# prashantraina/neural_raytracing

Measured on NVIDIA B200. Metric: rays_per_sec, higher is better.
Workload: dtype f16

## Files before the change

### neural_raytracing_b200/csrc/nrt_tc.cu

```cuda
#include <stdlib.h>

#include "tc_core.cuh"
#include "camera_math.cuh"

namespace tc {

template <int IN, int LAT, int OUT>
struct IoPlain {
  const float* x; const float* latent; float* out; int out_act;
  __device__ __forceinline__ void load(int64_t m, float* v) const {
#pragma unroll
    for (int j = 0; j < IN; ++j) v[j] = __ldg(x + m * IN + j);
#pragma unroll
    for (int j = 0; j < LAT; ++j) v[IN + j] = __ldg(latent + m * LAT + j);
  }
  __device__ __forceinline__ void store(int64_t m, const float* o) const {
#pragma unroll
    for (int j = 0; j < OUT; ++j) {
      float v = o[j];
      if (out_act == NRT_OUT_SIGMOID) v = 1.0f / (1.0f + __expf(-v));
      else if (out_act == NRT_OUT_SOFTPLUS) v = v > 20.0f ? v : __logf(1.0f + __expf(v));
      else if (out_act == NRT_OUT_TANH) v = tanhf(v);
      out[m * OUT + j] = v;
    }
  }
};

static inline int pow2_shift(int S) { int k = 0; while ((1 << k) < S) ++k; return (1 << k) == S ? k : -1; }
__device__ __forceinline__ int64_t ray_of(int64_t m, int S, int shift) { return shift >= 0 ? (m >> shift) : m / S; }

struct NoCam {};
struct WithCam { nrtcam::CamDev cam; int64_t r_off; };

template <int NLAT, bool CAM = false>
struct IoNerfFirst {
  const float* rays; const float* ts; const float* ts_per_ray; int S;
  float* sigma; void* latent; int fmt; int lat32; int s_shift;
  std::conditional_t<CAM, WithCam, NoCam> c;
  __device__ __forceinline__ void load(int64_t m, float* v) const {
    const int64_t ray = ray_of(m, S, s_shift);
    const int s = (int)(m - ray * S);
    const float t = ts_per_ray ? __ldg(ts_per_ray + m) : __ldg(ts + s);
    if constexpr (CAM) {
      float o[3], d[3];
      int view;
      nrtcam::cam_ray(c.cam, c.r_off + ray, o, d, &view);
      v[0] = o[0] + t * d[0]; v[1] = o[1] + t * d[1]; v[2] = o[2] + t * d[2];
    } else {
      const float* r = rays + ray * 6;
      v[0] = __ldg(r) + t * __ldg(r + 3);
      v[1] = __ldg(r + 1) + t * __ldg(r + 4);
      v[2] = __ldg(r + 2) + t * __ldg(r + 5);
    }
  }
  __device__ __forceinline__ void store(int64_t m, const float* o) const {
    sigma[m] = o[0];
    if (lat32) {
      float4* dst = reinterpret_cast<float4*>(latent) + (m >> 7) * (int64_t)(NLAT / 4 * 128) + (m & 127);
#pragma unroll
      for (int j = 0; j < NLAT / 4; ++j) dst[j * 128] = make_float4(o[1 + 4 * j], o[2 + 4 * j], o[3 + 4 * j], o[4 + 4 * j]);
      return;
    }
    uint4* dst = reinterpret_cast<uint4*>(latent) + (m >> 7) * (int64_t)(NLAT / 8 * 128) + (m & 127);
#pragma unroll
    for (int j = 0; j < NLAT / 8; ++j) {
      uint4 q;
      if (fmt == 0) {
        q.x = Elem<0>::pack(o[1 + 8 * j], o[2 + 8 * j]); q.y = Elem<0>::pack(o[3 + 8 * j], o[4 + 8 * j]);
        q.z = Elem<0>::pack(o[5 + 8 * j], o[6 + 8 * j]); q.w = Elem<0>::pack(o[7 + 8 * j], o[8 + 8 * j]);
      } else {
        q.x = Elem<1>::pack(o[1 + 8 * j], o[2 + 8 * j]); q.y = Elem<1>::pack(o[3 + 8 * j], o[4 + 8 * j]);
        q.z = Elem<1>::pack(o[5 + 8 * j], o[6 + 8 * j]); q.w = Elem<1>::pack(o[7 + 8 * j], o[8 + 8 * j]);
      }
      dst[j * 128] = q;
    }
  }
};

template <int NLAT, int LD, bool PACKED = false, bool CAM = false>
struct IoNerfSecond {
  const float* rays; const void* latent; const float* light_code; const int32_t* view_of_ray; int S;
  float* rgb; int fmt; int out_act; int lat32; int s_shift;
  std::conditional_t<CAM, WithCam, NoCam> c;
  __device__ __forceinline__ int dir_and_view(int64_t ray, float* d) const {
    if constexpr (CAM) {
      float o[3];
      int view;
      nrtcam::cam_ray(c.cam, c.r_off + ray, o, d, &view);
      return view;
    } else {
      const float* r = rays + ray * 6;
      d[0] = __ldg(r + 3); d[1] = __ldg(r + 4); d[2] = __ldg(r + 5);
      return view_of_ray ? __ldg(view_of_ray + ray) : 0;
    }
  }
  __device__ __forceinline__ void load(int64_t m, float* v) const {
    const int64_t ray = ray_of(m, S, s_shift);
    if (lat32) {
      const float4* src = reinterpret_cast<const float4*>(latent) + (m >> 7) * (int64_t)(NLAT / 4 * 128) + (m & 127);
#pragma unroll
      for (int j = 0; j < NLAT / 4; ++j) {
        const float4 q = __ldg(src + j * 128);
        v[4 * j] = q.x; v[4 * j + 1] = q.y; v[4 * j + 2] = q.z; v[4 * j + 3] = q.w;
      }
    } else {
      const uint4* src = reinterpret_cast<const uint4*>(latent) + (m >> 7) * (int64_t)(NLAT / 8 * 128) + (m & 127);
#pragma unroll
      for (int j = 0; j < NLAT / 8; ++j) {
        const uint4 q = __ldg(src + j * 128);
        const uint32_t w[4] = {q.x, q.y, q.z, q.w};
#pragma unroll
        for (int e = 0; e < 4; ++e) {
          if (fmt == 0) {
            v[8 * j + 2 * e] = Elem<0>::back((uint16_t)(w[e] & 0xffff)); v[8 * j + 2 * e + 1] = Elem<0>::back((uint16_t)(w[e] >> 16));
          } else {
            v[8 * j + 2 * e] = Elem<1>::back((uint16_t)(w[e] & 0xffff)); v[8 * j + 2 * e + 1] = Elem<1>::back((uint16_t)(w[e] >> 16));
          }
        }
      }
    }
    const int view = dir_and_view(ray, v + NLAT);
#pragma unroll
    for (int j = 0; j < LD; ++j) v[NLAT + 3 + j] = __ldg(light_code + (int64_t)view * LD + j);
  }
  static constexpr int kPackedPairs = PACKED ? NLAT / 2 : 0;
  __device__ __forceinline__ void load_packed(int64_t m, uint32_t* w, float* v) const {
    const int64_t ray = ray_of(m, S, s_shift);
    const uint4* src = reinterpret_cast<const uint4*>(latent) + (m >> 7) * (int64_t)(NLAT / 8 * 128) + (m & 127);
#pragma unroll
    for (int j = 0; j < NLAT / 8; ++j) {
      const uint4 q = __ldg(src + j * 128);
      w[4 * j] = q.x; w[4 * j + 1] = q.y; w[4 * j + 2] = q.z; w[4 * j + 3] = q.w;
    }
    const int view = dir_and_view(ray, v + NLAT);
#pragma unroll
    for (int j = 0; j < LD; ++j) v[NLAT + 3 + j] = __ldg(light_code + (int64_t)view * LD + j);
  }
  __device__ __forceinline__ void store(int64_t m, const float* o) const {
#pragma unroll
    for (int j = 0; j < 3; ++j) {
      float v = o[j];
      if (out_act == NRT_OUT_SIGMOID) v = 1.0f / (1.0f + __expf(-v));
      else if (out_act == NRT_OUT_TANH) v = tanhf(v);
      rgb[m * 3 + j] = v;
    }
  }
};

static long long* g_dbg_timeline = nullptr;
extern "C" void nrtdbg_set_timeline(long long* dev_buf) { g_dbg_timeline = dev_buf; }

#ifndef NRT_SPH_MAX
#define NRT_SPH_MAX 128
#endif
constexpr int kSphMax = NRT_SPH_MAX;
__device__ __forceinline__ float* sph_table() {
  __shared__ __align__(16) float tab[kSphMax * 13];
  return tab;
}
__device__ __forceinline__ void sph_fill(const SdfDev& sd) {
  if (sd.n > kSphMax) return;
  float* tab = sph_table();
  for (int e = threadIdx.x; e < sd.n * 13; e += blockDim.x) {
    const int i = e / 13, k = e - i * 13;
    float v;
    if (k == 12) v = __ldg(sd.radii + i);
    else {
      const int j = k >> 2, c = k & 3;
      v = c == 3 ? __ldg(sd.centers + i * 3 + j) : __ldg(sd.tfs + i * 9 + j * 3 + c) + (j == c ? 1.0f : 0.0f);
    }
    tab[k == 12 ? kSphMax * 12 + i : i * 12 + k] = v;
  }
}
template <bool APPROX = false>
__device__ __forceinline__ float sphere_smin_fast(const SdfDev& sd, float px, float py, float pz) {
  float sum = 0.0f;
  if (sd.n <= kSphMax) {
    const float4* rows = reinterpret_cast<const float4*>(sph_table());
    const float* rad = sph_table() + kSphMax * 12;
#pragma unroll 4
    for (int i = 0; i < sd.n; ++i) {
      const float4 a = rows[i * 3], b = rows[i * 3 + 1], c = rows[i * 3 + 2];
      const float q0 = fmaf(a.z, pz, fmaf(a.y, py, a.x * px)) - a.w;
      const float q1 = fmaf(b.z, pz, fmaf(b.y, py, b.x * px)) - b.w;
      const float q2 = fmaf(c.z, pz, fmaf(c.y, py, c.x * px)) - c.w;
      const float d2 = fmaf(q2, q2, fmaf(q1, q1, q0 * q0));
      if constexpr (APPROX) {
        float rs;
        asm("rsqrt.approx.ftz.f32 %0, %1;" : "=f"(rs) : "f"(fmaxf(d2, 1e-30f)));
        sum += tc::ex2_approx((rad[i] - d2 * rs) * 46.16624130844683f);
      } else {
        const float d = sqrtf(d2) - rad[i];
        sum += __expf(-32.0f * d);
      }
    }
    return -__logf(fmaxf(sum, 1e-4f)) * (1.0f / 32.0f);
  }
  for (int i = 0; i < sd.n; ++i) {
    const float* T = sd.tfs + i * 9;
    float q[3];
#pragma unroll
    for (int j = 0; j < 3; ++j) {
      const float t0 = __ldg(T + j * 3 + 0) + (j == 0 ? 1.0f : 0.0f);
      const float t1 = __ldg(T + j * 3 + 1) + (j == 1 ? 1.0f : 0.0f);
      const float t2 = __ldg(T + j * 3 + 2) + (j == 2 ? 1.0f : 0.0f);
      q[j] = fmaf(t2, pz, fmaf(t1, py, t0 * px)) - __ldg(sd.centers + i * 3 + j);
    }
    const float d = sqrtf(fmaf(q[2], q[2], fmaf(q[1], q[1], q[0] * q[0]))) - __ldg(sd.radii + i);
    sum += __expf(-32.0f * d);
  }
  return -__logf(fmaxf(sum, 1e-4f)) * (1.0f / 32.0f);
}

struct IoSdfEval {
  static constexpr int kSplitOut = 1;
  SdfDev sd; const float* p; float* out;
  __device__ __forceinline__ void cta_init() const { sph_fill(sd); }
  __device__ __forceinline__ void load(int64_t m, float* v) const {
    v[0] = __ldg(p + m * 3); v[1] = __ldg(p + m * 3 + 1); v[2] = __ldg(p + m * 3 + 2);
  }
  __device__ __forceinline__ void store(int64_t m, const float* o) const {
    out[m] = sphere_smin_fast(sd, __ldg(p + m * 3), __ldg(p + m * 3 + 1), __ldg(p + m * 3 + 2)) + o[0];
  }
};

__device__ __forceinline__ long long grab_ray(unsigned long long* counter, int64_t R, bool need) {
  const unsigned bal = __ballot_sync(0xffffffffu, need);
  if (bal == 0) return -1;
  const int lane = threadIdx.x & 31;
  unsigned long long base = 0;
  if (lane == __ffs(bal) - 1) base = atomicAdd(counter, (unsigned long long)__popc(bal));
  base = __shfl_sync(0xffffffffu, base, __ffs(bal) - 1);
  const long long r = (long long)base + __popc(bal & ((1u << lane) - 1u));
// ... 39 lines not shown
          s.d[0] = __ldg(rp + 3); s.d[1] = __ldg(rp + 4); s.d[2] = __ldg(rp + 5);
          s.t = t_start; s.it = 0; s.r = r;
          s.tmax = (MODE == TC_MARCH_SHADOW) ? __ldg(max_t_per_ray + r) : max_t;
        }
      }
    }
    if (s.r < 0) return false;
#pragma unroll
    for (int j = 0; j < 3; ++j) { s.p[j] = __fadd_rn(s.o[j], __fmul_rn(s.d[j], s.t)); x[j] = s.p[j]; }
    return true;
  }
  __device__ __forceinline__ void consume(State& s, const float* o) const {
    const float d = sphere_smin_fast<MODE != TC_MARCH_PRIMARY || ((NRT_MARCH_FAST & 2) != 0)>(sd, s.p[0], s.p[1], s.p[2]) + o[0];
    s.steps++;
    if (MODE == TC_MARCH_PRIMARY) {
      if (d <= eps) { depth[s.r] = s.t; flag[s.r] = 1; s.r = -1; }
      else { s.t += d; s.it++; }
    } else {
      s.t += d; s.it++;
      if (d < eps) { flag[s.r] = (s.t >= s.tmax) ? 1 : 0; s.r = -1; }
    }
  }
  __device__ __forceinline__ void finish(State& s) const {
    if (steps_done == nullptr) return;
    unsigned v = s.steps;
    for (int o = 16; o > 0; o >>= 1) v += __shfl_down_sync(0xffffffffu, v, o);
    if ((threadIdx.x & 31) == 0 && v) atomicAdd(steps_done, (unsigned long long)v);
  }
};

struct IoScanEval {
  static constexpr int kSoftplusForm = 3;
  __device__ __forceinline__ void cta_init() const { sph_fill(sd); }
  SdfDev sd;
  const float* rays; double step; int n1; float* val;
  __device__ __forceinline__ void point(int64_t m, float* p) const {
    const uint32_t ray = (uint32_t)m / (uint32_t)n1;
    const int k = (int)((uint32_t)m - ray * (uint32_t)n1);
    const float* rp = rays + (int64_t)ray * 6;
    const float t = (float)(step * (double)k);
#pragma unroll
    for (int j = 0; j < 3; ++j) p[j] = (k == 0) ? __ldg(rp + j) : __fadd_rn(__ldg(rp + j), __fmul_rn(t, __ldg(rp + 3 + j)));
  }
  __device__ __forceinline__ void load(int64_t m, float* x) const { point(m, x); }
  __device__ __forceinline__ void store(int64_t m, const float* o) const {
    float p[3];
    point(m, p);
    val[m] = sphere_smin_fast<true>(sd, p[0], p[1], p[2]) + o[0];
  }
};
__global__ void k_scan_argmin(const float* __restrict__ val, const float* __restrict__ rays, int64_t R, int n1, double step,
                              int32_t* __restrict__ best_idx, float* __restrict__ best_pos, float* __restrict__ min_val) {
  const int lane = threadIdx.x & 31;
  const int64_t r = ((int64_t)blockIdx.x * blockDim.x + threadIdx.x) >> 5;
  if (r >= R) return;
  const float* v = val + r * n1;
  float best = 3.0e38f;
  int idx = 0x7fffffff;
  for (int k = lane; k < n1; k += 32) {
    const float x = v[k];
    if (x < best) { best = x; idx = k; }
  }
  for (int o = 16; o > 0; o >>= 1) {
    const float ob = __shfl_xor_sync(0xffffffffu, best, o);
    const int oi = __shfl_xor_sync(0xffffffffu, idx, o);
    if (ob < best || (ob == best && oi < idx)) { best = ob; idx = oi; }
  }
  if (lane == 0) {
    best_idx[r] = idx;
    if (min_val) min_val[r] = best;
    const float tb = __fmul_rn((float)idx, (float)step);
    for (int j = 0; j < 3; ++j) best_pos[r * 3 + j] = __fadd_rn(rays[r * 6 + j], __fmul_rn(tb, rays[r * 6 + 3 + j]));
  }
}

template <class NET, class IO, int FMT, class SV = NoSave>
static int launch(const void* blob, const IO& io, int64_t M, cudaStream_t st, int tag = TAG_TC_MLP, SV sv = SV{}) {
  const size_t bytes = (size_t)NET::SMEM_BYTES + 256;
  auto kern = k_mlp_tc<NET, IO, FMT, SV>;
  NRT_CUDA(cudaFuncSetAttribute(kern, cudaFuncAttributeMaxDynamicSharedMemorySize, (int)bytes));
  const int64_t ntiles = (M + 127) / 128;
  const int grid = (int)std::min<int64_t>((ntiles + NET::NSLOT - 1) / NET::NSLOT, (int64_t)nrt_sm_count());
  NrtProfScope _ps(tag, st);
  kern<<<grid, NET::threads(NET::WPS), bytes, st>>>(reinterpret_cast<const uint8_t*>(blob) + NET::BLOB_OFF, io, M, g_dbg_timeline, sv);
  NRT_CUDA(cudaGetLastError());
  return NRT_OK;
}

using NetNerfFirst = Net<3, 0, 16, 128, 5, 3, 65, NRT_ACT_LEAKY_RELU>;
using NetNerfFirstR = Net<3, 0, 16, 128, 5, 3, 65, NRT_ACT_LEAKY_RELU, (NRT_BIAS_MMA & 4) != 0>;
using NetNerfSecondPT = Net<70, 0, 16, 64, 8, 3, 3, NRT_ACT_LEAKY_RELU>;
using NetNerfSecondLE = Net<115, 0, 16, 64, 8, 3, 3, NRT_ACT_LEAKY_RELU>;
using NetNeuralBsdf = Net<3, 0, 64, 96, 6, 3, 3, NRT_ACT_LEAKY_RELU>;
using NetOcc = Net<5, 0, 16, 64, 8, 3, 1, NRT_ACT_LEAKY_RELU>;
using NetPlainFirst = Net<3, 32, 16, 32, 5, 3, 33, NRT_ACT_LEAKY_RELU>;
using NetPlainSecond = Net<2, 64, 16, 32, 5, 3, 3, NRT_ACT_LEAKY_RELU>;
using NetSdfShift = Net<3, 0, 32, 128, 8, 3, 1, NRT_ACT_SOFTPLUS>;

template <class NET>
static bool matches(const MlpDev& d) {
  return d.in_size == NET::IN && d.latent == NET::LAT && d.freqs == NET::F && d.hidden == NET::H && d.L == NET::L &&
         d.skip == NET::SKIP && d.out == NET::OUT && d.act == NET::ACT;
}
template <class NET>
static bool matches(const nrt_mlp_t& m) {
  return m.in_size == NET::IN && m.latent_size == NET::LAT && m.freqs == NET::F && m.hidden == NET::H && m.num_layers == NET::L &&
         m.skip == NET::SKIP && m.out_size == NET::OUT && m.act == NET::ACT;
}

}

using namespace tc;

static int fmt_of(int prec) { return prec == NRT_PREC_BF16 ? 1 : 0; }

extern "C" int64_t nrt_mlp_tc_blob_bytes(const nrt_mlp_t* m, int prec) {
  NRT_REQUIRE(m != nullptr, "mlp descriptor is NULL");
  NRT_REQUIRE(prec == NRT_PREC_F16 || prec == NRT_PREC_BF16, "nrt_mlp_tc_blob_bytes: prec must be F16 or BF16");
  NRT_REQUIRE(m->num_layers >= 1 && m->num_layers <= NRT_MAX_LAYERS && m->hidden % 16 == 0, "unsupported MLP shape");
  if (matches<NetNerfFirst>(*m)) return (int64_t)NetNerfFirstR::BLOB_OFF + NetNerfFirstR::Y.bytes;
  const Layout y = make_layout(m->in_size, m->latent_size, m->freqs, m->hidden, m->num_layers, m->skip, m->out_size);
  return (int64_t)y.bytes;
}

extern "C" int nrt_mlp_pack_tc(const nrt_mlp_t* m, int prec, void* blob_out, void* stream) {
  MlpDev d;
  int rc = nrt_build_mlp_dev(m, &d);
  if (rc != NRT_OK) return rc;
  NRT_REQUIRE(prec == NRT_PREC_F16 || prec == NRT_PREC_BF16, "nrt_mlp_pack_tc: prec must be F16 or BF16");
  NRT_REQUIRE(blob_out != nullptr && ((uintptr_t)blob_out & 15) == 0, "blob_out must be 16-byte aligned");
  NRT_REQUIRE(d.hidden % 16 == 0, "hidden must be a multiple of 16");
  NrtProfScope _ps(TAG_TC_PACK, (cudaStream_t)stream);
  auto pack = [&](const Layout& y, const BiasRows& br, uint8_t* dst) {
    const int grid = std::min(nrt_cdiv(pack_tc_items(y), 256), 1184);
    if (fmt_of(prec) == 0) k_pack_tc<0><<<grid, 256, 0, (cudaStream_t)stream>>>(d, y, br, dst);
    else k_pack_tc<1><<<grid, 256, 0, (cudaStream_t)stream>>>(d, y, br, dst);
  };
  pack(make_layout(d.in_size, d.latent, d.freqs, d.hidden, d.L, d.skip, d.out), no_bias_rows(), (uint8_t*)blob_out);
  if (NetNerfFirstR::BLOB_OFF > 0 && matches<NetNerfFirst>(d))
    pack(NetNerfFirstR::Y, NetNerfFirstR::BR, (uint8_t*)blob_out + NetNerfFirstR::BLOB_OFF);
  NRT_CUDA(cudaGetLastError());
  return NRT_OK;
}

template <class NET>
static int forward_plain(const nrt_mlp_t* m, int prec, int out_act, const float* x, const float* latent, int64_t M,
                         float* out, cudaStream_t st) {
  IoPlain<NET::IN, NET::LAT, NET::OUT> io{x, latent, out, out_act};
  if (fmt_of(prec) == 0) return launch<NET, decltype(io), 0>(m->params_tc, io, M, st);
  return launch<NET, decltype(io), 1>(m->params_tc, io, M, st);
}
template <class NET>
static int forward_plain_save(const nrt_mlp_t* m, int prec, int out_act, const float* x, const float* latent, int64_t M,
                              float* out, float* acts, cudaStream_t st) {
  IoPlain<NET::IN, NET::LAT, NET::OUT> io{x, latent, out, out_act};
  SaveF32 sv{acts, M};
  if (fmt_of(prec) == 0) return launch<NET, decltype(io), 0, SaveF32>(m->params_tc, io, M, st, TAG_TC_MLP, sv);
  return launch<NET, decltype(io), 1, SaveF32>(m->params_tc, io, M, st, TAG_TC_MLP, sv);
}

int nrt_mlp_forward_tc_wide(const nrt_mlp_t* m, const MlpDev& d, int prec, int out_act, const float* x, int64_t M, float* out,
                            float* acts, cudaStream_t st, bool* handled);

int nrt_mlp_forward_tc(const nrt_mlp_t* m, int prec, int out_act, const float* x, const float* latent, int64_t M,
                       float* out, float* acts, cudaStream_t st) {
  MlpDev d;
  int rc = nrt_build_mlp_dev(m, &d);
// ... 192 lines not shown
```

### neural_raytracing_b200/csrc/tc_core.cuh

```cuda
#pragma once
#include <cuda_bf16.h>
#include <cuda_fp16.h>

#include <algorithm>
#include <type_traits>

#include "nrt_common.cuh"

namespace tc {

constexpr int kMaxOps = NRT_MAX_LAYERS + 3;

struct Layout {
  int split, XR, KRAW, KE, KX, KPH, FP, NOP;
  int n_ops;
  int opN[kMaxOps], opK[kMaxOps];
  int op_off[kMaxOps];
  int w_elems;
  int bias_off[kMaxOps];
  int bias_floats;
  int wout_f32_off;
  int basis_f32_off;
  int bytes;
};
// ... 836 lines not shown
#define NRT_MMA_WARP_PER_SLOT_STREAM 0
#endif
#ifndef NRT_SELF_ISSUE
#define NRT_SELF_ISSUE 0
#endif
  static constexpr bool SELF = NRT_SELF_ISSUE != 0 && STREAM && ACT == NRT_ACT_SOFTPLUS && ENC_CUDA && FUSE_OUT && NSLOT == 2;
  static constexpr int NMMA = SELF ? 0 : ((STREAM ? NRT_MMA_WARP_PER_SLOT_STREAM != 0 : NRT_MMA_WARP_PER_SLOT != 0) ? NSLOT : 1);
  static constexpr int threads(int wps) { return NWG * wps * 32 + 32 * NMMA; }
  static constexpr int max_op_bytes() {
    int m = 0;
    for (int o = 0; o < Y.n_ops; ++o) m = imax(m, Y.opN[o] * Y.opK[o] * 2);
    return m;
  }
  static constexpr int MAXOP = max_op_bytes();
  static constexpr int BIAS_BYTES = Y.bias_floats * 4;
  static constexpr int SMEM_BYTES = STREAM ? NSLOT * 2 * MAXOP + BIAS_BYTES : Y.bytes;
  static constexpr bool FITS_SMEM = SMEM_BYTES <= kSmemBudget;
};

constexpr int kEpiThreads = 128;

template <class NET, int FMT, int ST, int PART = 0, bool BMMA = false, int ZLO = 0>
__device__ __forceinline__ void issue_stage(uint32_t b_addr, uint32_t dD, uint32_t aU, uint32_t aE, uint64_t* done_bar) {
  constexpr Layout Y = NET::Y;
  constexpr uint32_t N = (uint32_t)Y.opN[ST];
  constexpr uint32_t idesc = (1u << 4) | ((uint32_t)FMT << 7) | ((uint32_t)FMT << 10) | ((N >> 3) << 17) |
                             ((uint32_t)(128 >> 4) << 24);
  constexpr uint32_t lbo = N * 16, sbo = 128;
  constexpr int kch = Y.opK[ST] / 16;
  constexpr int k_u = (ST >= 2 && ST < NET::STAGES - 1) ? NET::H / 16 : ((NET::INPLACE && ST == 1) ? 0 : kch);
  if (elect_one()) {
    const uint64_t bd0 = make_desc(NET::STREAM ? b_addr : b_addr + (uint32_t)Y.op_off[ST] * 2u, lbo, sbo);
    constexpr bool kBiasChunk = BMMA && !NET::BIAS_ROWS && ST > 0 && ST < NET::END_STAGE;
    constexpr bool kBiasChunk8 = BMMA && NET::BIAS_ROWS && NET::BR.bk8_off[ST] >= 0;
    constexpr bool kFromZero = ST == 0 || (BMMA && NET::BIAS_ROWS && NET::BR.bk8_off[ST] < 0);
    if constexpr (kBiasChunk) {
      static_assert(NET::BIAS_MMA && N == (uint32_t)NET::H, "bias K-chunks: hidden-width MMA layers of a resident blob");
      mma_ts(dD, (uint32_t)NET::ONES_COL, make_desc(b_addr + (uint32_t)NET::BK_OFF + (uint32_t)(ST - 1) * N * 32u, lbo, sbo), idesc, 0u);
    }
    if constexpr (kBiasChunk8) {
      static_assert(!NET::STREAM, "bias chunks of a resident blob");
      mma_ts(dD, (uint32_t)NET::ONES_COL, make_desc(b_addr + (uint32_t)NET::BR.bk8_off[ST] * 2u, lbo, sbo), idesc, 0u);
    }
#pragma unroll
    for (int kc = 0; kc < kch; ++kc) {
      if (PART == 1 && kc >= k_u / 2 && kc < k_u) continue;
      if (PART == 2 && (kc < k_u / 2 || kc >= k_u)) continue;
      uint32_t a;
      if constexpr (ST == 0) {
        constexpr int xch = NET::XR / 16;
        static_assert(ZLO < xch, "the chunk with the non-latent x_lo columns stays");
        if (kc >= xch && kc < xch + ZLO) continue;
        const uint32_t hi = NET::INPLACE ? aE : aU, lo = NET::INPLACE ? aU : aE;
        a = (kc >= xch && kc < 2 * xch) ? (lo + (kc - xch) * 8) : (hi + (kc % xch) * 8);
      } else {
        a = (kc < k_u) ? (aU + kc * 8) : (aE + (kc - k_u) * 8);
      }
      mma_ts(dD, a, bd0 + (uint64_t)((kc * 2 * lbo) >> 4), idesc, (!kFromZero || kc > 0) ? 1u : 0u);
    }
    if (PART != 1) tc_commit(done_bar);
  }
  __syncwarp();
}
template <class NET, int FMT, int PART = 0, bool BMMA = false, int ZLO = 0>
__device__ __forceinline__ void issue_stage_dyn(int st, uint32_t b_addr, uint32_t dD, uint32_t aU, uint32_t aE,
                                                uint64_t* done_bar) {
#define NRT_STAGE_CASE(S) case S: if constexpr (S < NET::STAGES && (PART == 0 || S >= 2)) issue_stage<NET, FMT, S, PART, BMMA, ZLO>(b_addr, dD, aU, aE, done_bar); break;
  switch (st) {
    NRT_STAGE_CASE(0) NRT_STAGE_CASE(1) NRT_STAGE_CASE(2) NRT_STAGE_CASE(3) NRT_STAGE_CASE(4) NRT_STAGE_CASE(5)
    NRT_STAGE_CASE(6) NRT_STAGE_CASE(7) NRT_STAGE_CASE(8) NRT_STAGE_CASE(9) NRT_STAGE_CASE(10) NRT_STAGE_CASE(11)
    NRT_STAGE_CASE(12) NRT_STAGE_CASE(13) NRT_STAGE_CASE(14) NRT_STAGE_CASE(15) NRT_STAGE_CASE(16) NRT_STAGE_CASE(17)
    NRT_STAGE_CASE(18) NRT_STAGE_CASE(19) NRT_STAGE_CASE(20) NRT_STAGE_CASE(21) NRT_STAGE_CASE(22)
    default: break;
  }
#undef NRT_STAGE_CASE
}
__device__ __forceinline__ void stream_op(uint8_t* dst, const uint8_t* src, uint32_t bytes, uint64_t* bar) {
  mbar_expect_tx(bar, bytes);
  for (uint32_t off = 0; off < bytes; off += 32768u) bulk_g2s(dst + off, src + off, min(32768u, bytes - off), bar);
}

template <class T, class = void> struct PackedPairsOf { static constexpr int value = 0; };
template <class T> struct PackedPairsOf<T, std::void_t<decltype(T::kPackedPairs)>> { static constexpr int value = T::kPackedPairs; };
template <class T, class = void> struct HasCtaInit : std::false_type {};
template <class T> struct HasCtaInit<T, std::void_t<decltype(&T::cta_init)>> : std::true_type {};
template <class T, class = void> struct IsIterative : std::false_type {};
template <class T> struct IsIterative<T, std::void_t<typename T::State>> : std::true_type {};
struct NoState {};
template <class T, class = void> struct StateOf { using type = NoState; };
template <class T> struct StateOf<T, std::void_t<typename T::State>> { using type = typename T::State; };

__device__ __forceinline__ void named_bar_sync(int id, int nthreads) {
  asm volatile("bar.sync %0, %1;" ::"r"(id), "r"(nthreads) : "memory");
}

#ifdef NRT_MAXNREG
#define NRT_KMLP_BOUNDS(T) __maxnreg__(((65536 / (T)) / 8 * 8) > 255 ? 255 : ((65536 / (T)) / 8 * 8))
#else
#define NRT_KMLP_BOUNDS(T) __launch_bounds__(T, 1)
#endif
template <class NET, class IO, int FMT, class SV = NoSave, int WPS = NET::WPS>
__global__ void NRT_KMLP_BOUNDS(NET::threads(WPS))
k_mlp_tc(const uint8_t* __restrict__ blob, IO io, int64_t M, long long* __restrict__ dbg, SV sv = SV{}) {
  constexpr int EPI = WPS * 32;
  static_assert(NET::FITS_TMEM, "network does not fit in TMEM");
  static_assert(NET::FITS_SMEM, "stage buffers do not fit in shared memory");
  constexpr int kDbgIt0 = 4, kDbgIts = 4;
  auto stamp = [&](int it, int st, int slot, int k) {
    if (dbg != nullptr && slot < 2 && blockIdx.x == 0 && it >= kDbgIt0 && it < kDbgIt0 + kDbgIts)
      dbg[(((it - kDbgIt0) * NET::STAGES + st) * 2 + slot) * 8 + k] = clock64();
  };
  using E = Elem<FMT>;
  constexpr Layout Y = NET::Y;
  constexpr int H = NET::H, IN = NET::IN, LAT = NET::LAT, F = NET::F, L = NET::L;
  constexpr int NSLOT = NET::NSLOT;
  extern __shared__ __align__(128) uint8_t smem[];
  constexpr bool STREAM = NET::STREAM;
  uint16_t* sW = reinterpret_cast<uint16_t*>(smem);
  const float* sBias = reinterpret_cast<const float*>(smem + (STREAM ? (size_t)NSLOT * 2 * NET::MAXOP : (size_t)Y.w_elems * 2));
  __shared__ __align__(8) uint64_t bar_w;
  __shared__ __align__(8) uint64_t bar_wfull[3][2];
  __shared__ uint32_t s_opoff[NET::STAGES], s_opbytes[NET::STAGES];
  __shared__ __align__(8) uint64_t bar_ready[3];
  __shared__ __align__(8) uint64_t bar_ready_a[3];
  __shared__ __align__(8) uint64_t bar_done[3];
  constexpr bool KSPLIT = NET::KSPLIT && WPS == 4 && !SV::kOn && !SV::kF32;
#ifndef NRT_SOFTPLUS_FULLROW
#define NRT_SOFTPLUS_FULLROW 0
#endif
#ifndef NRT_SOFTPLUS_PIPE
#define NRT_SOFTPLUS_PIPE 1
#endif
  constexpr bool kPipeRow = NRT_SOFTPLUS_PIPE != 0 && SoftplusOf<IO>::value != 0 && NET::ACT == NRT_ACT_SOFTPLUS && !KSPLIT &&
                            !SV::kOn && !SV::kF32;
  constexpr bool kFullRow = NRT_SOFTPLUS_FULLROW != 0 && !kPipeRow && NET::ACT == NRT_ACT_SOFTPLUS && !KSPLIT && !SV::kOn && !SV::kF32;
  __shared__ uint32_t tmem_base_s;
  __shared__ uint32_t s_bias[NET::STAGES];
  constexpr bool ITER = IsIterative<IO>::value;
  constexpr bool BMMA = NET::BIAS_MMA && !KSPLIT && WPS == 4 && !SV::kOn && !SV::kF32;
  static_assert(BMMA || !NET::BIAS_ROWS, "the render layout has no fp32 biases to pre-load");
  constexpr int kPP = (!ITER && !NET::SPLIT && !SV::kOn && !SV::kF32 && LAT == 0 && NET::ACT == NRT_ACT_LEAKY_RELU) ? PackedPairsOf<IO>::value : 0;
  constexpr int ZLO = (NRT_BIAS_MMA & 2) ? 2 * kPP / 16 : 0;
  __shared__ volatile uint32_t s_slot_live[3];
  __shared__ uint32_t s_warp_live[3][4];

  const int tid = threadIdx.x;
  const int warp = tid >> 5;
  constexpr bool SELF = NET::SELF;
  const int mma_id = SELF ? -1 : warp - NET::NWG * WPS;
  const bool is_mma_warp = SELF ? warp == 0 : mma_id == 0;
  __shared__ uint32_t s_issue_lock;
  const int64_t ntiles = (M + 127) / 128;
  if constexpr (HasCtaInit<IO>::value) io.cta_init();
  if (tid < NET::STAGES) {
    s_bias[tid] = (uint32_t)Y.bias_off[tid];
    s_opoff[tid] = (uint32_t)Y.op_off[tid] * 2;
    s_opbytes[tid] = (uint32_t)(Y.opN[tid] * Y.opK[tid] * 2);
  }

  if (tid == 0) {
    s_slot_live[0] = 1; s_slot_live[1] = 1; s_slot_live[2] = 1;
    s_issue_lock = 0;
    mbar_init(&bar_w, 1);
    for (int s = 0; s < 3; ++s) {
      mbar_init(&bar_ready[s], EPI); mbar_init(&bar_done[s], 1); mbar_init(&bar_ready_a[s], EPI);
      mbar_init(&bar_wfull[s][0], 1); mbar_init(&bar_wfull[s][1], 1);
    }
    asm volatile("fence.mbarrier_init.release.cluster;" ::: "memory");
  }
  __syncthreads();
  if (is_mma_warp) {
    asm volatile("tcgen05.alloc.cta_group::1.sync.aligned.shared::cta.b32 [%0], 512;" ::"r"(smem_u32(&tmem_base_s)) : "memory");
    asm volatile("tcgen05.relinquish_alloc_permit.cta_group::1.sync.aligned;" ::: "memory");
    if ((tid & 31) == 0) {
      if (STREAM) {
        mbar_expect_tx(&bar_w, (uint32_t)NET::BIAS_BYTES);
        bulk_g2s(smem + (size_t)NSLOT * 2 * NET::MAXOP, blob + (size_t)Y.w_elems * 2, (uint32_t)NET::BIAS_BYTES, &bar_w);
      } else {
        mbar_expect_tx(&bar_w, (uint32_t)Y.bytes);
        constexpr uint32_t kChunk = 32768;
        for (uint32_t off = 0; off < (uint32_t)Y.bytes; off += kChunk) {
          const uint32_t n = min(kChunk, (uint32_t)Y.bytes - off);
          bulk_g2s(smem + off, blob + off, n, &bar_w);
        }
      }
    }
  }
  tc_fence_before();
  __syncthreads();
  tc_fence_after();
  if (tmem_base_s != 0u) __trap();
  constexpr uint32_t tmem = 0u;
  if constexpr (BMMA) {
    if (warp < 4) {
      const uint32_t one = (uint32_t)one16<FMT>();
      const uint32_t r[8] = {one | (one << 16), one, 0u, 0u, 0u, 0u, 0u, 0u};
      TmemIO<8>::st(tmem + ((uint32_t)(warp * 32) << 16) + (uint32_t)NET::ONES_COL, r);
      tc_wait_st();
    }
    tc_fence_before();
    __syncthreads();
    tc_fence_after();
  }
  mbar_wait(&bar_w, 0);

  if (mma_id >= 0) {
    constexpr int NMMA = NET::NMMA;
    constexpr bool OWN = NMMA == NSLOT;
    auto mine = [&](int slot) { return slot % (NMMA > 0 ? NMMA : 1) == mma_id; };
#ifndef NRT_MMA_ALTERNATE
#define NRT_MMA_ALTERNATE 0
#endif
    constexpr bool ALT = NRT_MMA_ALTERNATE != 0 && !OWN && NSLOT == 2 && !KSPLIT;
    int turn = 0;
    bool live[3];
    auto is_ready = [&](int slot, uint64_t* bar, uint32_t parity) {
      if constexpr (OWN) { mbar_wait(bar, parity); return true; }
      else if constexpr (ALT) {
        if (slot != turn && live[turn]) return false;
        mbar_wait(bar, parity);
        turn = slot ^ 1;
        return true;
      }
      else return mbar_test(bar, parity);
    };
// ... 82 lines not shown
            stream_op(smem + (size_t)(slot * 2 + nb) * NET::MAXOP, blob + s_opoff[st[slot]], s_opbytes[st[slot]],
                      &bar_wfull[slot][nb]);
          }
          __syncwarp();
        }
      }
#ifndef NRT_MMA_POLL_SLEEP_NS
#define NRT_MMA_POLL_SLEEP_NS 0
#endif
      if (NRT_MMA_POLL_SLEEP_NS > 0 && !progressed) __nanosleep(NRT_MMA_POLL_SLEEP_NS);
    }
  } else {
    const int slot = warp / WPS;
    const int half = (WPS == 8) ? ((warp >> 2) & 1) : 0;
    const bool primary = half == 0;
    const int lane_row = (warp & 3) * 32 + (tid & 31);
    constexpr int HW = (WPS == 8) ? H / 2 : H;
    if (slot < NSLOT) {
      const uint32_t lane_off = ((uint32_t)((warp & 3) * 32)) << 16;
      const uint32_t base = tmem + slot * NET::COLS + lane_off;
      const uint32_t dD = base, aU = base + NET::DC, aE = base + NET::DC + NET::UC;
      uint32_t n_done = 0;
      int it_dbg = 0;
#ifndef NRT_DBG_LANE
#define NRT_DBG_LANE 0
#endif
      auto estamp = [&](int st, int k) { if (lane_row == NRT_DBG_LANE) stamp(it_dbg, st, slot, k); };
      typename StateOf<IO>::type state;
      if constexpr (ITER) io.init(state);
      const bool leader = SELF && (warp % WPS) == 0;
      int st_mma = NET::FIRST_STAGE;
      uint32_t n_ready_l = 0, n_issued_l = 0;
      const uint32_t sW_addr_l = smem_u32(sW);
      if constexpr (SELF) {
        if (leader) {
          if (elect_one())
            stream_op(smem + (size_t)(slot * 2) * NET::MAXOP, blob + s_opoff[NET::FIRST_STAGE], s_opbytes[NET::FIRST_STAGE],
                      &bar_wfull[slot][0]);
          __syncwarp();
        }
      }
      auto self_issue = [&]() {
        if constexpr (SELF) {
          if (leader) {
            mbar_wait(&bar_ready[slot], n_ready_l & 1); n_ready_l++;
            const uint32_t b = n_issued_l & 1;
            mbar_wait(&bar_wfull[slot][b], (n_issued_l >> 1) & 1);
            if ((tid & 31) == 0) {
              while (atomicCAS(&s_issue_lock, 0u, 1u) != 0u) __nanosleep(64);
            }
            __syncwarp();
            tc_fence_after();
            if ((tid & 31) == 0) stamp(it_dbg, st_mma, slot, 1);
            const uint32_t base0 = tmem + slot * NET::COLS;
            issue_stage_dyn<NET, FMT>(st_mma, sW_addr_l + (uint32_t)((slot * 2 + b) * NET::MAXOP), base0, base0 + NET::DC,
                                      base0 + NET::DC + NET::UC, &bar_done[slot]);
            if ((tid & 31) == 0) {
              stamp(it_dbg, st_mma, slot, 2);
              __threadfence_block();
              atomicExch(&s_issue_lock, 0u);
            }
            if (++st_mma == NET::END_STAGE) st_mma = NET::FIRST_STAGE;
            n_issued_l++;
            if (elect_one()) {
              const uint32_t nb = n_issued_l & 1;
              stream_op(smem + (size_t)(slot * 2 + nb) * NET::MAXOP, blob + s_opoff[st_mma], s_opbytes[st_mma], &bar_wfull[slot][nb]);
            }
            __syncwarp();
          }
        }
      };
      auto self_drain = [&]() {
        if constexpr (SELF) {
          if (leader) mbar_wait(&bar_wfull[slot][n_issued_l & 1], (n_issued_l >> 1) & 1);
        }
      };
#ifndef NRT_SLOT_STAGGER
#define NRT_SLOT_STAGGER 900
#endif
      if (NRT_SLOT_STAGGER > 0 && slot > 0) {
        const long long t_start = clock64();
        while (clock64() - t_start < (long long)slot * NRT_SLOT_STAGGER) {}
      }
      for (int64_t t0 = (int64_t)blockIdx.x * NSLOT;; t0 += (int64_t)gridDim.x * NSLOT, ++it_dbg) {
        int64_t m = 0;
        bool valid;
        float x[IN + LAT];
        uint32_t pw[kPP > 0 ? kPP : 1];
        if constexpr (ITER) {
          valid = primary ? io.next(state, x) : false;
          const unsigned bal = __ballot_sync(0xffffffffu, valid);
          if (primary && (tid & 31) == 0) s_warp_live[slot][warp & 3] = bal;
          named_bar_sync(1 + slot, EPI);
          const bool any = (s_warp_live[slot][0] | s_warp_live[slot][1] | s_warp_live[slot][2] | s_warp_live[slot][3]) != 0;
          if (!any) {
            if (lane_row == 0) s_slot_live[slot] = 0;
            mbar_arrive(&bar_ready[slot]);
            self_drain();
            break;
          }
        } else {
          const int64_t tile = t0 + slot;
          if (tile >= ntiles) { self_drain(); break; }
          m = tile * 128 + lane_row;
          valid = m < M;
          if constexpr (kPP > 0) {
            if (valid && primary) io.load_packed(m, pw, x);
          } else {
            if (valid && primary) io.load(m, x);
          }
        }
        if (!primary) {
          if constexpr (!NET::ENC_CUDA) {
            mbar_arrive(&bar_ready[slot]);
            mbar_wait(&bar_done[slot], n_done & 1); n_done++;
          }
          mbar_arrive(&bar_ready[slot]);
          self_issue();
        } else {
        uint32_t ex[NET::XR / 2];
        {
          if (!valid) {
#pragma unroll
            for (int j = 0; j < IN + LAT; ++j) x[j] = 0.0f;
          }
          uint32_t ax[NET::KX / 2];
#pragma unroll
          for (int j = 0; j < NET::KX / 2; ++j) { ax[j] = 0; ex[j] = 0; }
          if constexpr (NET::SPLIT) {
            uint16_t v[16];
#pragma unroll
            for (int j = 0; j < 16; ++j) v[j] = 0;
            uint16_t a[2 * IN];
#pragma unroll
            for (int j = 0; j < IN; ++j) {
              const uint16_t hi = E::cvt(x[j]);
              const uint16_t lo = E::cvt(x[j] - E::back(hi));
              v[j] = hi; v[IN + j] = lo; v[2 * IN + j] = hi;
              const float ax_ = act_fast<NET::ACT>(x[j]);
              const uint16_t ahi = E::cvt(ax_);
              a[j] = ahi; a[IN + j] = E::cvt(ax_ - E::back(ahi));
            }
            if constexpr (NET::BIAS_ROWS) {
#pragma unroll
              for (int t = 0; t < 3; ++t) v[NET::BR.row + t] = one16<FMT>();
            }
#pragma unroll
            for (int j = 0; j < 8; ++j) ax[j] = (uint32_t)v[2 * j] | ((uint32_t)v[2 * j + 1] << 16);
#pragma unroll
            for (int j = 0; j < IN; ++j) ex[j] = (uint32_t)a[2 * j] | ((uint32_t)a[2 * j + 1] << 16);
            if constexpr (NET::BIAS_ROWS) {
#pragma unroll
              for (int t = 0; t < 3; ++t) ex[(NET::BR.row + t) / 2] |= (uint32_t)one16<FMT>() << (16 * ((NET::BR.row + t) & 1));
            }
            tmem_store<NET::KX / 2>(aU, ax);
            if constexpr (NET::INPLACE) tmem_store<NET::XR / 2>(aE, ax);
            else tmem_store<NET::XR / 2>(aE, ex);
          } else {
            uint32_t lx[NET::XR / 2];
#pragma unroll
            for (int j = 0; j < NET::XR / 2; ++j) lx[j] = 0;
#pragma unroll
            for (int j = 0; j < (IN + 1) / 2; ++j) {
              if (kPP > 0 && j < kPP) {
                ax[j] = valid ? pw[j] : 0u;
                if constexpr (!NET::INPLACE) ex[j] = leaky_packed<FMT>(ax[j]);
                continue;
              }
              const float xa = x[2 * j], xb = (2 * j + 1 < IN) ? x[2 * j + 1 < IN ? 2 * j + 1 : 0] : 0.0f;
              ax[j] = E::pack(xa, xb);
              const float ha = E::back((uint16_t)(ax[j] & 0xffffu)), hb = E::back((uint16_t)(ax[j] >> 16));
              lx[j] = E::pack(xa - ha, xb - hb);
              ex[j] = E::pack(act_fast<NET::ACT>(xa), (2 * j + 1 < IN) ? act_fast<NET::ACT>(xb) : 0.0f);
            }
            if constexpr (NET::INPLACE) { tmem_store<NET::XR / 2>(aE, ax); tmem_store<NET::XR / 2>(aU, lx); }
            else { tmem_store<NET::XR / 2>(aU, ax); tmem_store<NET::XR / 2>(aE, lx); }
          }
          if constexpr (SV::kOn) {
            static_assert(!ITER, "activation tiles are saved by the tile policies only");
            uint16_t* rr = tile_row_ptr(sv.enc_raw, m >> 7, NET::KE + kTileRowsExtra, lane_row);
            uint16_t* ra = tile_row_ptr(sv.enc_act, m >> 7, NET::KE + kTileRowsExtra, lane_row);
            save_cols<NET::KX / 2>(rr, 0, ax);
            if constexpr (!NET::INPLACE) save_cols<NET::XR / 2>(ra, 0, ex);
            rr[tile_elem(NET::KE)] = one16<FMT>();
            ra[tile_elem(NET::KE)] = one16<FMT>();
          }
          if constexpr (LAT > 0) {
            uint32_t lr[LAT / 2], la[LAT / 2];
#pragma unroll
            for (int j = 0; j < LAT / 2; ++j) {
              lr[j] = E::pack(x[IN + 2 * j], x[IN + 2 * j + 1]);
              la[j] = E::pack(act_fast<NET::ACT>(x[IN + 2 * j]), act_fast<NET::ACT>(x[IN + 2 * j + 1]));
            }
            tmem_store<LAT / 2>(aU + (NET::XR + 2 * F) / 2, lr);
            tmem_store<LAT / 2>(aE + (NET::XR + 2 * F) / 2, la);
            if constexpr (SV::kOn) {
              save_cols<LAT / 2>(tile_row_ptr(sv.enc_raw, m >> 7, NET::KE + kTileRowsExtra, lane_row), NET::XR + 2 * F, lr);
              save_cols<LAT / 2>(tile_row_ptr(sv.enc_act, m >> 7, NET::KE + kTileRowsExtra, lane_row), NET::XR + 2 * F, la);
            }
          }
          if constexpr (!NET::ENC_CUDA) {
            tc_wait_st();
            tc_fence_before();
            mbar_arrive(&bar_ready[slot]);
          }
        }
        {
          uint32_t ph[F];
          if constexpr (NET::ENC_CUDA) {
            const float* sB = sBias + Y.basis_f32_off;
#pragma unroll
            for (int f = 0; f < F; ++f) {
              float p = x[0] * sB[f];
#pragma unroll
              for (int j = 1; j < IN; ++j) p = fmaf(x[j], sB[j * NET::FP + f], p);
              ph[f] = __float_as_uint(p);
            }
          } else {
            mbar_wait(&bar_done[slot], n_done & 1); n_done++;
            tc_fence_after();
            tmem_load<F>(dD, ph);
            tc_wait_ld();
            if constexpr (!NET::INPLACE) tmem_store<NET::XR / 2>(aE, ex);
          }
          if constexpr (!BMMA) preload_bias<H>(dD, sBias + s_bias[1]);
          uint32_t sr[F / 2], cr[F / 2], sa[F / 2], ca[F / 2];
#pragma unroll
          for (int j = 0; j < F / 2; ++j) {
            float s0, c0, s1, c1;
            sincos_fast(__uint_as_float(ph[2 * j]), &s0, &c0);
            sincos_fast(__uint_as_float(ph[2 * j + 1]), &s1, &c1);
            sr[j] = E::pack(s0, s1); cr[j] = E::pack(c0, c1);
            sa[j] = E::pack(act_fast<NET::ACT>(s0), act_fast<NET::ACT>(s1));
            ca[j] = E::pack(act_fast<NET::ACT>(c0), act_fast<NET::ACT>(c1));
          }
          if constexpr (NET::INPLACE) {
            tmem_store<F / 2>(aE + NET::XR / 2, sr);
            tmem_store<F / 2>(aE + NET::XR / 2 + F / 2, cr);
          } else {
            tmem_store<F / 2>(aU + NET::XR / 2, sr);
            tmem_store<F / 2>(aU + NET::XR / 2 + F / 2, cr);
            tmem_store<F / 2>(aE + NET::XR / 2, sa);
            tmem_store<F / 2>(aE + NET::XR / 2 + F / 2, ca);
          }
          if constexpr (SV::kOn) {
            uint16_t* rr = tile_row_ptr(sv.enc_raw, m >> 7, NET::KE + kTileRowsExtra, lane_row);
            uint16_t* ra = tile_row_ptr(sv.enc_act, m >> 7, NET::KE + kTileRowsExtra, lane_row);
            save_cols<F / 2>(rr, NET::XR, sr);
            save_cols<F / 2>(rr, NET::XR + F, cr);
            if constexpr (!NET::INPLACE) {
              save_cols<F / 2>(ra, NET::XR, sa);
              save_cols<F / 2>(ra, NET::XR + F, ca);
            }
          }
          tc_wait_st();
          tc_fence_before();
          mbar_arrive(&bar_ready[slot]);
          self_issue();
        }
        }
        constexpr int NHID = NET::FUSE_OUT ? L : L + 1;
#pragma unroll 1
        for (int st = 0; st < NHID; ++st) {
          estamp(2 + st, 3);
          mbar_wait(&bar_done[slot], n_done & 1); n_done++;
          tc_fence_after();
          estamp(2 + st, 4);
          if constexpr (!KSPLIT) estamp(2 + st, 5);
          const int coff = half * HW;
          auto pre = [&]() {
            if constexpr (NET::INPLACE) {
              if (st == 0 && primary) {
                static_assert(NET::KE % 16 == 0, "encoding width");
#pragma unroll
                for (int c = 0; c < NET::EC / 8; ++c) {
                  uint32_t e[8];
                  TmemIO<8>::ld(aE + 8 * c, e);
                  tc_wait_ld();
#pragma unroll
                  for (int j = 0; j < 8; ++j) e[j] = leaky_packed<FMT>(e[j]);
                  TmemIO<8>::st(aE + 8 * c, e);
                  if constexpr (SV::kOn)
                    save_cols<8>(tile_row_ptr(sv.enc_act, m >> 7, NET::KE + kTileRowsExtra, lane_row), 16 * c, e);
                }
              }
            }
            if constexpr (BMMA) {
            } else if (st < L) preload_bias<HW>(dD + coff, sBias + s_bias[2 + st] + coff);
            else {
              constexpr int N0 = (WPS != 8 || NET::NOP < HW) ? NET::NOP : HW, N1 = (WPS == 8 && NET::NOP > HW) ? NET::NOP - HW : 0;
              if (primary) preload_bias<N0>(dD, sBias + s_bias[NET::STAGES - 1]);
              else if constexpr (N1 > 0) preload_bias<N1>(dD + HW, sBias + s_bias[NET::STAGES - 1] + HW);
            }
          };
          if constexpr (KSPLIT) {
            long long* d = nullptr;
            if (dbg != nullptr && lane_row == 0 && slot < 2 && blockIdx.x == 0 && it_dbg >= kDbgIt0 && it_dbg < kDbgIt0 + kDbgIts)
              d = dbg + (((it_dbg - kDbgIt0) * NET::STAGES + 2 + st) * 2 + slot) * 8;
            convert_row_split<NET::ACT, FMT, HW>(dD, aU, &bar_ready_a[slot], &bar_ready[slot], pre, d ? d + 5 : nullptr,
                                                 d ? d + 6 : nullptr);
            estamp(2 + st, 7);
          } else {
          if constexpr (SV::kOn)
            convert_row<NET::ACT, FMT, HW, true>(dD + coff, aU + coff / 2,
                tile_row_ptr(sv.acts, (int64_t)st * sv.ntiles + (m >> 7), H + kTileRowsExtra, lane_row), coff, primary ? H : -1,
                sv.masks + (int64_t)st * (H / 32) * (sv.ntiles * 128) + m, sv.ntiles * 128);
          else if constexpr (SV::kF32)
            convert_row_savef32<NET::ACT, FMT, HW>(dD + coff, aU + coff / 2,
                                                   valid ? sv.acts + ((int64_t)st * H) * sv.M + m : nullptr, sv.M);
          else if constexpr (kPipeRow) {
            long long* d = nullptr;
#ifdef NRT_DBG_CONV
            if (dbg != nullptr && lane_row == NRT_DBG_LANE && slot < 2 && blockIdx.x == 0 && it_dbg >= kDbgIt0 && it_dbg < kDbgIt0 + kDbgIts)
              d = dbg + (((it_dbg - kDbgIt0) * NET::STAGES + 2 + st) * 2 + slot) * 8 + 3;
#endif
            convert_row_pipe<FMT, HW, SoftplusOf<IO>::value>(dD + coff, aU + coff / 2, pre, d);
          }
          else if constexpr (kFullRow)
            convert_row_full<NET::ACT, FMT, HW>(dD + coff, aU + coff / 2, pre);
          else
            convert_row<NET::ACT, FMT, HW>(dD + coff, aU + coff / 2);
          if constexpr (!(kFullRow || kPipeRow) || SV::kOn || SV::kF32) pre();
          estamp(2 + st, 6);
          tc_wait_st();
          tc_fence_before();
          mbar_arrive(&bar_ready[slot]);
          estamp(2 + st, 7);
          self_issue();
          }
        }
        if (!primary) {
          mbar_wait(&bar_done[slot], n_done & 1); n_done++;
          tc_fence_after();
          tc_fence_before();
        } else if constexpr (NET::FUSE_OUT) {
          mbar_wait(&bar_done[slot], n_done & 1); n_done++;
          tc_fence_after();
          float o[NET::OUT];
#pragma unroll
          for (int j = 0; j < NET::OUT; ++j) o[j] = sBias[s_bias[NET::STAGES - 1] + j];
          if constexpr (SV::kOn)
            convert_row_out<NET::ACT, FMT, H, NET::OUT, true>(dD, sBias + Y.wout_f32_off, o,
                tile_row_ptr(sv.acts, (int64_t)L * sv.ntiles + (m >> 7), H + kTileRowsExtra, lane_row),
                sv.masks + (int64_t)L * (H / 32) * (sv.ntiles * 128) + m, sv.ntiles * 128);
          else if constexpr (SV::kF32)
            convert_row_out_savef32<NET::ACT, FMT, H, NET::OUT>(dD, sBias + Y.wout_f32_off, o,
                                                                  valid ? sv.acts + ((int64_t)L * H) * sv.M + m : nullptr, sv.M);
          else
            convert_row_out<NET::ACT, FMT, H, NET::OUT, false, kPipeRow || (NRT_SOFTPLUS_POLY != 0)>(dD, sBias + Y.wout_f32_off, o);
          if constexpr (ITER) { if (valid) io.consume(state, o); }
          else { if (valid) io.store(m, o); }
          tc_fence_before();
        } else {
          mbar_wait(&bar_done[slot], n_done & 1); n_done++;
          tc_fence_after();
          constexpr int OC = (NET::OUT + 7) / 8 * 8;
          uint32_t acc[OC];
          tmem_load<OC>(dD, acc);
          tc_wait_ld();
          float o[NET::OUT];
#pragma unroll
          for (int j = 0; j < NET::OUT; ++j) o[j] = __uint_as_float(acc[j]);
          if constexpr (ITER) { if (valid) io.consume(state, o); }
          else { if (valid) io.store(m, o); }
          tc_fence_before();
        }
      }
      if constexpr (ITER) { if (primary) io.finish(state); }
    }
  }
  tc_fence_before();
  __syncthreads();
  if (is_mma_warp) asm volatile("tcgen05.dealloc.cta_group::1.sync.aligned.b32 %0, 512;" ::"r"(tmem) : "memory");
}


}
```

Before: 13.16 million.

## Software-pipeline next tile's input fetch and encoding across the first NeRF MLP epilogue

For the bias-row render layout (NeRF first network), the input loads for the next tile are prefetched one iteration ahead. The next tile's encoding (hi/lo splits, activations, sin/cos features) is computed before waiting on the current tile's output MMA, and the encoding is stored to tensor memory alongside the output tmem load, so the next MMA chain can be signalled earlier. This hides global-load latency and encoding ALU work behind the tail of the previous tile, at the cost of more live registers (the Fetch and Enc structs) and a more complex slot schedule. It also adds a debug option that restricts timeline stamping to one kernel tag, plus optional boundary stamps.

Result: faster. 13.77 million, median of 6 (+4.6%).

```diff
diff --git a/neural_raytracing_b200/csrc/nrt_tc.cu b/neural_raytracing_b200/csrc/nrt_tc.cu
--- a/neural_raytracing_b200/csrc/nrt_tc.cu
+++ b/neural_raytracing_b200/csrc/nrt_tc.cu
@@ -37,21 +37,27 @@
   const float* rays; const float* ts; const float* ts_per_ray; int S;
   float* sigma; void* latent; int fmt; int lat32; int s_shift;
   std::conditional_t<CAM, WithCam, NoCam> c;
-  __device__ __forceinline__ void load(int64_t m, float* v) const {
+  struct Fetch { float t, o[3], d[3]; };
+  __device__ __forceinline__ void fetch(int64_t m, Fetch& f) const {
     const int64_t ray = ray_of(m, S, s_shift);
     const int s = (int)(m - ray * S);
-    const float t = ts_per_ray ? __ldg(ts_per_ray + m) : __ldg(ts + s);
+    f.t = ts_per_ray ? __ldg(ts_per_ray + m) : __ldg(ts + s);
     if constexpr (CAM) {
-      float o[3], d[3];
       int view;
-      nrtcam::cam_ray(c.cam, c.r_off + ray, o, d, &view);
-      v[0] = o[0] + t * d[0]; v[1] = o[1] + t * d[1]; v[2] = o[2] + t * d[2];
+      nrtcam::cam_ray(c.cam, c.r_off + ray, f.o, f.d, &view);
     } else {
       const float* r = rays + ray * 6;
-      v[0] = __ldg(r) + t * __ldg(r + 3);
-      v[1] = __ldg(r + 1) + t * __ldg(r + 4);
-      v[2] = __ldg(r + 2) + t * __ldg(r + 5);
-    }
+#pragma unroll
+      for (int j = 0; j < 3; ++j) { f.o[j] = __ldg(r + j); f.d[j] = __ldg(r + 3 + j); }
+    }
+  }
+  __device__ __forceinline__ static void point(const Fetch& f, float* v) {
+    v[0] = f.o[0] + f.t * f.d[0]; v[1] = f.o[1] + f.t * f.d[1]; v[2] = f.o[2] + f.t * f.d[2];
+  }
+  __device__ __forceinline__ void load(int64_t m, float* v) const {
+    Fetch f;
+    fetch(m, f);
+    point(f, v);
   }
   __device__ __forceinline__ void store(int64_t m, const float* o) const {
     sigma[m] = o[0];
@@ -148,7 +154,9 @@
 };
 
 static long long* g_dbg_timeline = nullptr;
+static int g_dbg_timeline_tag = -1;
 extern "C" void nrtdbg_set_timeline(long long* dev_buf) { g_dbg_timeline = dev_buf; }
+extern "C" void nrtdbg_set_timeline_tag(int tag) { g_dbg_timeline_tag = tag; }
 
 #ifndef NRT_SPH_MAX
 #define NRT_SPH_MAX 128
@@ -354,7 +362,8 @@
   const int64_t ntiles = (M + 127) / 128;
   const int grid = (int)std::min<int64_t>((ntiles + NET::NSLOT - 1) / NET::NSLOT, (int64_t)nrt_sm_count());
   NrtProfScope _ps(tag, st);
-  kern<<<grid, NET::threads(NET::WPS), bytes, st>>>(reinterpret_cast<const uint8_t*>(blob) + NET::BLOB_OFF, io, M, g_dbg_timeline, sv);
+  long long* dbg = g_dbg_timeline_tag < 0 || g_dbg_timeline_tag == tag ? g_dbg_timeline : nullptr;
+  kern<<<grid, NET::threads(NET::WPS), bytes, st>>>(reinterpret_cast<const uint8_t*>(blob) + NET::BLOB_OFF, io, M, dbg, sv);
   NRT_CUDA(cudaGetLastError());
   return NRT_OK;
 }
diff --git a/neural_raytracing_b200/csrc/tc_core.cuh b/neural_raytracing_b200/csrc/tc_core.cuh
--- a/neural_raytracing_b200/csrc/tc_core.cuh
+++ b/neural_raytracing_b200/csrc/tc_core.cuh
@@ -942,6 +942,8 @@
 
 template <class T, class = void> struct PackedPairsOf { static constexpr int value = 0; };
 template <class T> struct PackedPairsOf<T, std::void_t<decltype(T::kPackedPairs)>> { static constexpr int value = T::kPackedPairs; };
+template <class T, class D, class = void> struct FetchOf { using type = D; };
+template <class T, class D> struct FetchOf<T, D, std::void_t<typename T::Fetch>> { using type = typename T::Fetch; };
 template <class T, class = void> struct HasCtaInit : std::false_type {};
 template <class T> struct HasCtaInit<T, std::void_t<decltype(&T::cta_init)>> : std::true_type {};
 template <class T, class = void> struct IsIterative : std::false_type {};
@@ -1001,6 +1003,12 @@
   static_assert(BMMA || !NET::BIAS_ROWS, "the render layout has no fp32 biases to pre-load");
   constexpr int kPP = (!ITER && !NET::SPLIT && !SV::kOn && !SV::kF32 && LAT == 0 && NET::ACT == NRT_ACT_LEAKY_RELU) ? PackedPairsOf<IO>::value : 0;
   constexpr int ZLO = (NRT_BIAS_MMA & 2) ? 2 * kPP / 16 : 0;
+#ifndef NRT_FIRST_PIPE
+#define NRT_FIRST_PIPE 1
+#endif
+  constexpr bool PIPE = NRT_FIRST_PIPE != 0 && NET::BIAS_ROWS && !ITER;
+  static_assert(!PIPE || (BMMA && NET::SPLIT && NET::ENC_CUDA && !NET::FUSE_OUT && !NET::INPLACE && LAT == 0 && WPS == 4),
+                "NRT_FIRST_PIPE: NeRFLE.first's render layout (split fp32 encoding, bias rows, an MMA output layer)");
   __shared__ volatile uint32_t s_slot_live[3];
   __shared__ uint32_t s_warp_live[3][4];
 
@@ -1249,6 +1257,107 @@
         const long long t_start = clock64();
         while (clock64() - t_start < (long long)slot * NRT_SLOT_STAGGER) {}
       }
+#ifdef NRT_DBG_BOUNDARY
+      auto bstamp = [&](int it, int k) { if (lane_row == NRT_DBG_LANE) stamp(it, 0, slot, k); };
+      auto bstamp_dep = [&](int it, int k, float v) { if (lane_row == NRT_DBG_LANE && __float_as_uint(v) != 0xffffffffu) stamp(it, 0, slot, k); };
+#else
+      auto bstamp = [&](int, int) {};
+      auto bstamp_dep = [&](int, int, float) {};
+#endif
+      struct Inputs { float v[IN + LAT]; };
+      using Pre = typename FetchOf<IO, Inputs>::type;
+      struct Enc { uint32_t ax[NET::KX / 2], ex[NET::XR / 2], sr[F / 2], cr[F / 2], sa[F / 2], ca[F / 2]; };
+      const int64_t tstride = (int64_t)gridDim.x * NSLOT;
+      Pre pre;
+      bool pre_ok = false;
+      auto fetch = [&](int64_t mm) {
+        if constexpr (PIPE) {
+          pre_ok = mm < M;
+          if (pre_ok) {
+            if constexpr (std::is_same_v<Pre, Inputs>) io.load(mm, pre.v);
+            else io.fetch(mm, pre);
+          }
+        }
+      };
+      auto inputs = [&](float* xi) {
+        if (PIPE && pre_ok) {
+          if constexpr (std::is_same_v<Pre, Inputs>) {
+#pragma unroll
+            for (int j = 0; j < IN; ++j) xi[j] = pre.v[j];
+          } else io.point(pre, xi);
+        } else {
+#pragma unroll
+          for (int j = 0; j < IN; ++j) xi[j] = 0.0f;
+        }
+      };
+      auto encode = [&](const float* xi, Enc& e) {
+        if constexpr (PIPE) {
+        uint16_t v[16];
+#pragma unroll
+        for (int j = 0; j < 16; ++j) v[j] = 0;
+        uint16_t a[2 * IN];
+#pragma unroll
+        for (int j = 0; j < IN; ++j) {
+          const uint16_t hi = E::cvt(xi[j]);
+          const uint16_t lo = E::cvt(xi[j] - E::back(hi));
+          v[j] = hi; v[IN + j] = lo; v[2 * IN + j] = hi;
+          const float ax_ = act_fast<NET::ACT>(xi[j]);
+          const uint16_t ahi = E::cvt(ax_);
+          a[j] = ahi; a[IN + j] = E::cvt(ax_ - E::back(ahi));
+        }
+#pragma unroll
+        for (int t = 0; t < 3; ++t) v[NET::BR.row + t] = one16<FMT>();
+#pragma unroll
+        for (int j = 0; j < NET::XR / 2; ++j) e.ex[j] = 0;
+#pragma unroll
+        for (int j = 0; j < NET::KX / 2; ++j) e.ax[j] = (uint32_t)v[2 * j] | ((uint32_t)v[2 * j + 1] << 16);
+#pragma unroll
+        for (int j = 0; j < IN; ++j) e.ex[j] = (uint32_t)a[2 * j] | ((uint32_t)a[2 * j + 1] << 16);
+#pragma unroll
+        for (int t = 0; t < 3; ++t) e.ex[(NET::BR.row + t) / 2] |= (uint32_t)one16<FMT>() << (16 * ((NET::BR.row + t) & 1));
+        const float* sB = sBias + Y.basis_f32_off;
+        uint32_t ph[F];
+#pragma unroll
+        for (int f = 0; f < F; ++f) {
+          float p = xi[0] * sB[f];
+#pragma unroll
+          for (int j = 1; j < IN; ++j) p = fmaf(xi[j], sB[j * NET::FP + f], p);
+          ph[f] = __float_as_uint(p);
+        }
+#pragma unroll
+        for (int j = 0; j < F / 2; ++j) {
+          float s0, c0, s1, c1;
+          sincos_fast(__uint_as_float(ph[2 * j]), &s0, &c0);
+          sincos_fast(__uint_as_float(ph[2 * j + 1]), &s1, &c1);
+          e.sr[j] = E::pack(s0, s1); e.cr[j] = E::pack(c0, c1);
+          e.sa[j] = E::pack(act_fast<NET::ACT>(s0), act_fast<NET::ACT>(s1));
+          e.ca[j] = E::pack(act_fast<NET::ACT>(c0), act_fast<NET::ACT>(c1));
+        }
+        }
+      };
+      auto enc_store = [&](const Enc& e) {
+        tmem_store<NET::KX / 2>(aU, e.ax);
+        tmem_store<NET::XR / 2>(aE, e.ex);
+        tmem_store<F / 2>(aU + NET::XR / 2, e.sr);
+        tmem_store<F / 2>(aU + NET::XR / 2 + F / 2, e.cr);
+        tmem_store<F / 2>(aE + NET::XR / 2, e.sa);
+        tmem_store<F / 2>(aE + NET::XR / 2 + F / 2, e.ca);
+      };
+      if constexpr (PIPE) {
+        const int64_t tile = (int64_t)blockIdx.x * NSLOT + slot;
+        if (tile < ntiles) {
+          fetch(tile * 128 + lane_row);
+          float xi[IN];
+          inputs(xi);
+          Enc e;
+          encode(xi, e);
+          enc_store(e);
+          tc_wait_st();
+          tc_fence_before();
+          mbar_arrive(&bar_ready[slot]);
+          fetch((tile + tstride) * 128 + lane_row);
+        }
+      }
       for (int64_t t0 = (int64_t)blockIdx.x * NSLOT;; t0 += (int64_t)gridDim.x * NSLOT, ++it_dbg) {
         int64_t m = 0;
         bool valid;
@@ -1271,13 +1380,16 @@
           if (tile >= ntiles) { self_drain(); break; }
           m = tile * 128 + lane_row;
           valid = m < M;
-          if constexpr (kPP > 0) {
+          if constexpr (PIPE) {
+          } else if constexpr (kPP > 0) {
             if (valid && primary) io.load_packed(m, pw, x);
           } else {
             if (valid && primary) io.load(m, x);
-          }
-        }
-        if (!primary) {
+            if (valid) bstamp_dep(it_dbg, 5, x[0]);
+          }
+        }
+        if constexpr (PIPE) {
+        } else if (!primary) {
           if constexpr (!NET::ENC_CUDA) {
             mbar_arrive(&bar_ready[slot]);
             mbar_wait(&bar_done[slot], n_done & 1); n_done++;
@@ -1421,8 +1533,10 @@
             }
           }
           tc_wait_st();
+          bstamp(it_dbg, 6);
           tc_fence_before();
           mbar_arrive(&bar_ready[slot]);
+          bstamp(it_dbg, 7);
           self_issue();
         }
         }
@@ -1496,6 +1610,16 @@
           self_issue();
           }
         }
+        const bool has_next = PIPE && t0 + slot + tstride < ntiles;
+        Enc en;
+        if constexpr (PIPE) {
+          if (has_next) {
+            float xi[IN];
+            inputs(xi);
+            bstamp_dep(it_dbg + 1, 5, xi[0]);
+            encode(xi, en);
+          }
+        }
         if (!primary) {
           mbar_wait(&bar_done[slot], n_done & 1); n_done++;
           tc_fence_after();
@@ -1523,13 +1647,28 @@
           tc_fence_after();
           constexpr int OC = (NET::OUT + 7) / 8 * 8;
           uint32_t acc[OC];
+          bstamp(it_dbg, 3);
           tmem_load<OC>(dD, acc);
-          tc_wait_ld();
+          if constexpr (PIPE) {
+            if (has_next) enc_store(en);
+            tc_wait_ld();
+            if (has_next) {
+              tc_wait_st();
+              bstamp(it_dbg + 1, 6);
+              tc_fence_before();
+              mbar_arrive(&bar_ready[slot]);
+              bstamp(it_dbg + 1, 7);
+              fetch((t0 + slot + 2 * tstride) * 128 + lane_row);
+            }
+          } else {
+            tc_wait_ld();
+          }
           float o[NET::OUT];
 #pragma unroll
           for (int j = 0; j < NET::OUT; ++j) o[j] = __uint_as_float(acc[j]);
           if constexpr (ITER) { if (valid) io.consume(state, o); }
           else { if (valid) io.store(m, o); }
+          bstamp(it_dbg, 4);
           tc_fence_before();
         }
       }
```
